# Twinklebear/tray_rust

Hardware: NVIDIA H100
Metric: Mrays/s (primary+secondary) (higher is better)
Workload: dtype f32

## Files before the change

include/trb.h:

```cpp
#ifndef TRB_H
#define TRB_H

#include <stdint.h>
#include <stddef.h>

#ifdef __cplusplus
extern "C" {
#endif

#define TRB_ABI_VERSION 4u

typedef enum trb_status {
    TRB_OK = 0,
    TRB_INVALID_ARG = 1,
    TRB_CUDA = 2,
    TRB_OOM = 3,
    TRB_UNSUPPORTED = 4,
    TRB_IO = 5,
    TRB_NO_DEVICE = 6,
    TRB_NCCL = 7
} trb_status;


typedef struct trb_keyframe {
// ... 590 lines not shown
                                     uint32_t* pixel_spp, trb_stats* stats);

trb_status trb_adaptive_schedule(const trb_adaptive* adaptive, uint32_t* min_spp, uint32_t* max_spp, uint32_t* step,
                                 uint32_t* max_per_pixel);

trb_status trb_host_adaptive_decide(const trb_adaptive* adaptive, const float* lum, size_t n, uint32_t* samples_taken,
                                    float* avg);


trb_status trb_block_list(const trb_scene* scene, uint32_t block_start, uint32_t block_count,
                          uint32_t* n_out, uint32_t* xy_pairs, uint32_t capacity);

trb_status trb_scene_get_bvh(const trb_scene* scene, int which, uint32_t* n_nodes, trb_bvh_node* nodes,
                             uint32_t* n_ordered, uint32_t* ordered);

trb_status trb_scene_get_transform(const trb_scene* scene, uint32_t inst, float* mat16, float* inv16);

trb_status trb_scene_get_filter_table(const trb_scene* scene, float* table256);


trb_status trb_host_build_bvh(const float* boxes6, uint32_t n, uint32_t max_geom, uint32_t* n_nodes,
                              trb_bvh_node* nodes, uint32_t* ordered);

trb_status trb_build_bvh(int device, const float* boxes6, uint32_t n, uint32_t max_geom, uint32_t* n_nodes,
                         trb_bvh_node* nodes, uint32_t* ordered);

trb_status trb_build_bvh_device(int device, const float* d_boxes6, uint32_t n, uint32_t max_geom, uint32_t* d_n_nodes,
                                trb_bvh_node* d_nodes, uint32_t* d_ordered, void* cuda_stream);

trb_status trb_host_keyframe_transform(const trb_keyframe* kf, float* mat16, float* inv16);
// ... 30 lines not shown
```

tray_rust_b200/_ffi.py:

```python
import ctypes as C
import os

_HERE = os.path.dirname(os.path.abspath(__file__))
REPO = os.path.dirname(_HERE)

TRB_ABI_VERSION = 4
TRB_OK, TRB_INVALID_ARG, TRB_CUDA, TRB_OOM, TRB_UNSUPPORTED, TRB_IO, TRB_NO_DEVICE, TRB_NCCL = range(8)
INST_RECEIVER, INST_EMITTER_AREA, INST_EMITTER_POINT = 0, 1, 2
SHAPE_NONE, SHAPE_SPHERE, SHAPE_DISK, SHAPE_RECT, SHAPE_MESH = 0, 1, 2, 3, 4
MAT_MATTE, MAT_PLASTIC, MAT_METAL, MAT_SPECULAR_METAL, MAT_GLASS, MAT_ROUGH_GLASS, MAT_MERL = range(7)
FILTER_MITCHELL_NETRAVALI, FILTER_GAUSSIAN = 0, 1
INTEGRATOR_PATH, INTEGRATOR_WHITTED, INTEGRATOR_NORMALS_DEBUG = 0, 1, 2
RENDER_STATS, RENDER_NO_UPDATE, RENDER_REFERENCE_SHADOW, RENDER_MEGAKERNEL, RENDER_TIME_TRACE = 1, 2, 4, 8, 16
QUERY_CLAMP = 32
BXDF_REFLECTION, BXDF_TRANSMISSION, BXDF_DIFFUSE, BXDF_GLOSSY, BXDF_SPECULAR = 1, 2, 4, 8, 16
BXDF_ALL = 31
MISS = 0xFFFFFFFF
BVH_LEAF = 0x80000000
MERL_TABLE_FLOATS = 90 * 90 * 180 * 3

u32, f32 = C.c_uint32, C.c_float


class Keyframe(C.Structure):
# ... 236 lines not shown
BSDF_SAMPLE_QUERY_DTYPE = np.dtype([("wo", "<f4", 3), ("bxdf", "<u4"), ("u", "<f4", 2), ("u_comp", "<f4"), ("pad", "<u4")])
BSDF_SAMPLE_DTYPE = np.dtype([("f", "<f4", 3), ("pdf", "<f4"), ("wi", "<f4", 3), ("sampled", "<u4")])
LIGHT_QUERY_DTYPE = np.dtype([("p", "<f4", 3), ("time", "<f4"), ("u", "<f4", 2), ("light", "<u4"), ("pad", "<u4")])
LIGHT_SAMPLE_DTYPE = np.dtype([("li", "<f4", 3), ("pdf", "<f4"), ("wi", "<f4", 3), ("delta", "<u4"), ("shadow", QUERY_RAY_DTYPE)])
LIGHT_PDF_QUERY_DTYPE = np.dtype([("p", "<f4", 3), ("time", "<f4"), ("wi", "<f4", 3), ("light", "<u4")])
EMIT_QUERY_DTYPE = np.dtype([("w", "<f4", 3), ("time", "<f4"), ("n", "<f4", 3), ("inst", "<u4")])
KEYFRAME_DTYPE = np.dtype([("translation", "<f4", 3), ("rotation", "<f4", 4), ("scaling", "<f4", 3)])
COLOR_KEY_DTYPE = np.dtype([("rgba", "<f4", 4), ("time", "<f4")])
AOV_SAMPLE_DTYPE = np.dtype([("albedo", "<f4", 3), ("depth", "<f4"), ("n", "<f4", 3), ("inst", "<u4")])
MATERIAL_DTYPE = np.dtype([("type", "<u4"), ("c0", "<f4", 3), ("c1", "<f4", 3), ("roughness", "<f4"), ("eta", "<f4"), ("merl", "<u4"),
                           ("tex", "<u4", 4)])

TRB_SYMBOLS = [
    "trb_scene_create", "trb_scene_load_json", "trb_scene_destroy", "trb_scene_info", "trb_scene_update_frame",
    "trb_render", "trb_render_device", "trb_intersect", "trb_intersect_device", "trb_camera_rays",
    "trb_render_samples", "trb_film_to_srgb8", "trb_block_list", "trb_scene_get_bvh", "trb_scene_get_transform",
    "trb_scene_get_filter_table", "trb_last_error", "trb_abi_version", "trb_desc_load_json", "trb_desc_free",
    "trb_host_build_bvh", "trb_host_keyframe_transform", "trb_host_animated_transform", "trb_host_animated_color", "trb_host_quad_check", "trb_selftest_box", "trb_launch_count", "trb_scene_trace_time", "trb_scene_check_error", "trb_scene_set_option", "trb_write_png",
    "trb_nccl_unique_id", "trb_comm_create", "trb_comm_destroy", "trb_comm_info", "trb_comm_reduce_film", "trb_render_sharded",
    "trb_group_create", "trb_group_load_json", "trb_group_render", "trb_group_scene", "trb_group_destroy",
    "trb_render_adaptive", "trb_render_samples_adaptive", "trb_adaptive_schedule", "trb_host_adaptive_decide",
    "trb_render_adaptive_device", "trb_render_sharded_adaptive", "trb_group_render_adaptive",
    "trb_intersect_records", "trb_intersect_records_device", "trb_occluded", "trb_occluded_device",
    "trb_illumination", "trb_illumination_device",
    "trb_bsdf_eval", "trb_bsdf_eval_device", "trb_bsdf_sample", "trb_bsdf_sample_device", "trb_light_sample", "trb_light_sample_device",
    "trb_light_pdf", "trb_light_pdf_device", "trb_emitted", "trb_emitted_device", "trb_scene_lights",
    "trb_film_write", "trb_film_write_device", "trb_camera_rays_device", "trb_host_film_to_srgb8",
    "trb_build_bvh", "trb_build_bvh_device",
    "trb_scene_update_mesh", "trb_scene_update_mesh_device", "trb_scene_refit_mesh", "trb_scene_refit_mesh_device",
    "trb_scene_update_keyframes", "trb_scene_update_keyframes_device", "trb_scene_update_color_keys", "trb_scene_update_materials",
    "trb_scene_replace_objects", "trb_scene_replace_meshes", "trb_scene_replace_meshes_device",
# ... 93 lines not shown
                                                 C.POINTER(DenoiseMomentsGradientOutput)]
    lib.trb_denoise_moments_gradient_device.argtypes = [vp, vp, C.POINTER(DenoiseFrame), C.POINTER(DenoiseGradientParams), u32,
                                                        C.POINTER(DenoiseMomentsGradientOutput), vp]
    lib.trb_render_adaptive.argtypes = [vp, C.POINTER(RenderCfg), C.POINTER(Adaptive), vp, vp, C.POINTER(Stats)]
    lib.trb_render_samples_adaptive.argtypes = [vp, C.POINTER(RenderCfg), C.POINTER(Adaptive), sz, vp, vp, C.POINTER(Stats)]
    lib.trb_render_adaptive_device.argtypes = [vp, C.POINTER(RenderCfg), C.POINTER(Adaptive), vp, vp, vp, vp]
    lib.trb_render_adaptive_aov.argtypes = [vp, C.POINTER(RenderCfg), C.POINTER(Adaptive), vp, C.POINTER(AovFilm), vp, C.POINTER(Stats)]
    lib.trb_render_adaptive_aov_device.argtypes = [vp, C.POINTER(RenderCfg), C.POINTER(Adaptive), vp, C.POINTER(AovFilm), vp, vp, vp]
    lib.trb_render_samples_adaptive_aov.argtypes = [vp, C.POINTER(RenderCfg), C.POINTER(Adaptive), sz, vp, vp, vp, C.POINTER(Stats)]
    lib.trb_adaptive_schedule.argtypes = [C.POINTER(Adaptive)] + [C.POINTER(u32)] * 4
    lib.trb_host_adaptive_decide.argtypes = [C.POINTER(Adaptive), vp, sz, C.POINTER(u32), C.POINTER(f32)]
    lib.trb_film_to_srgb8.argtypes = [vp, vp, vp]
    lib.trb_host_film_to_srgb8.argtypes = [u32, u32, vp, vp]
    lib.trb_block_list.argtypes = [vp, u32, u32, C.POINTER(u32), vp, u32]
    lib.trb_scene_get_bvh.argtypes = [vp, C.c_int, C.POINTER(u32), vp, C.POINTER(u32), vp]
    lib.trb_scene_get_transform.argtypes = [vp, u32, vp, vp]
    lib.trb_scene_get_filter_table.argtypes = [vp, vp]
    lib.trb_desc_load_json.argtypes = [C.c_char_p, u32, u32, u32, C.POINTER(C.POINTER(SceneDesc))]
    lib.trb_desc_free.argtypes = [C.POINTER(SceneDesc)]
    lib.trb_desc_free.restype = None
    lib.trb_host_build_bvh.argtypes = [vp, u32, u32, C.POINTER(u32), vp, vp]
    lib.trb_build_bvh.argtypes = [C.c_int, vp, u32, u32, C.POINTER(u32), vp, vp]
    lib.trb_build_bvh_device.argtypes = [C.c_int, vp, u32, u32, vp, vp, vp, vp]
    lib.trb_host_keyframe_transform.argtypes = [C.POINTER(Keyframe), vp, vp]
    lib.trb_host_animated_transform.argtypes = [C.POINTER(SceneDesc), u32, u32, f32, vp, vp]
    lib.trb_host_animated_color.argtypes = [C.POINTER(SceneDesc), u32, u32, f32, vp]
    lib.trb_host_quad_check.argtypes = [vp, u32, vp, u32, C.POINTER(u32), C.POINTER(C.c_uint64), C.POINTER(C.c_uint64)]
    lib.trb_selftest_box.argtypes = [u32, u32, C.POINTER(C.c_uint64)]
    lib.trb_launch_count.restype = C.c_uint64
    lib.trb_scene_trace_time.argtypes = [vp, C.POINTER(f32), C.POINTER(u32)]
# ... 26 lines not shown
```

tray_rust_b200/api.py:

```python
import ctypes as C

import numpy as np

from . import _ffi as F


class TrbError(RuntimeError):
    def __init__(self, status, msg):
        super().__init__("trb status %d: %s" % (status, msg))
        self.status = status


def _cfg(spp=0, sample_first=0, sample_count=0, block_start=0, block_count=0, current_frame=0, seed=1, flags=0,
         shard_index=0, shard_count=0, shard_chunk=0):
    return F.RenderCfg(spp, sample_first, sample_count, block_start, block_count, current_frame, seed, flags,
                       shard_index, shard_count, shard_chunk)


def adaptive_schedule(min_spp, max_spp):
    lib = F.load_trb()
    out = [F.u32() for _ in range(4)]
    rc = lib.trb_adaptive_schedule(C.byref(F.Adaptive(min_spp, max_spp)), *(C.byref(x) for x in out))
    if rc != F.TRB_OK:
        raise TrbError(rc, (lib.trb_last_error() or b"").decode())
# ... 537 lines not shown
            n = section.n_meshes
            meshes = (F.Mesh * max(1, n))()
            for i in range(n):
                k = section.keep[i]
                meshes[i] = section.meshes[i] if k == F.MESH_NEW else self._desc.meshes[k]
            desc.meshes, desc.n_meshes = meshes, n
        desc._keep = (self._desc, objects, section, meshes, materials)
        self._desc = desc
        w, hh, spp, nb, ni, nl = (F.u32() for _ in range(6))
        self._check(self._lib.trb_scene_info(self._h, *(C.byref(x) for x in (w, hh, spp, nb, ni, nl))))
        self.width, self.height, self.spp, self.total_blocks, self.n_instances, self.n_lights = (x.value for x in (w, hh, spp, nb, ni, nl))

    def set_option(self, name, value):
        self._check(self._lib.trb_scene_set_option(self._h, name.encode(), int(value)))

    def check_error(self):
        self._check(self._lib.trb_scene_check_error(self._h))

    def trace_time(self):
        ms, n = F.f32(), F.u32()
        self._check(self._lib.trb_scene_trace_time(self._h, C.byref(ms), C.byref(n)))
        return ms.value, n.value

    def render_samples(self, **kw):
        cfg = _cfg(**kw)
        n = self._n_samples(cfg)
        out = np.zeros(n, F.SAMPLE_DTYPE)
        st = F.Stats()
        self._check(self._lib.trb_render_samples(self._h, C.byref(cfg), n, F.ptr(out), C.byref(st)))
        return out, st
# ... 291 lines not shown
```

tray_rust_b200/csrc/trb_api.cu:

```cuda
#include <chrono>
#include <dlfcn.h>
#include <nccl.h>
#include <cstdio>
#include <cstdlib>
#include <memory>
#include <thread>
#include <tuple>
#include <cub/device/device_radix_sort.cuh>
#include "trb_host.h"
#include "trb_kernels.cuh"
#include "trb_bvh_build.cuh"
#include "trb_denoise.cuh"

using namespace trbh;

namespace {

thread_local std::string g_error;
unsigned long long g_launches = 0;
trb_status fail(trb_status s, const std::string& msg) { g_error = msg; return s; }

#define CU(call)                                                                                                   \
    do {                                                                                                           \
        cudaError_t e_ = (call);                                                                                   \
// ... 21 lines not shown
        if (e != cudaSuccess) return e;
        ptrs.push_back(d);
        *out = static_cast<T*>(d);
        return e;
    }
    void release(const void* p) {
        for (size_t i = 0; i < ptrs.size(); ++i)
            if (ptrs[i] == p) { cudaFree(ptrs[i]); ptrs[i] = ptrs.back(); ptrs.pop_back(); return; }
    }
};

struct HostMesh {
    std::vector<trb_bvh_node> nodes;
    std::vector<uint32_t> order;
    Box3 bounds;
    uint32_t n_verts = 0;
    bool narrow = true;
    size_t pair_cap = 0;
    bool stale = false;
    uint32_t* d_refit = nullptr;
};

uint32_t pow2_ceil(uint32_t v) { uint32_t p = 1; while (p < v) p <<= 1; return p; }

float bits_f(uint32_t u) { float f; std::memcpy(&f, &u, 4); return f; }
constexpr uint32_t QUAD_EMPTY_HOST = 0xffffffffu;
bool pack_pairs(const std::vector<trb_bvh_node>& in, std::vector<trb::DPair>& out, trb::DBvh& hdr, bool wide = false) {
    std::vector<uint32_t> rec_of(in.size(), 0);
    uint32_t n_rec = 0;
    for (size_t i = 0; i < in.size(); ++i) if (!(in[i].b & TRB_BVH_LEAF)) rec_of[i] = n_rec++;
    bool ok = n_rec < (1u << 30);
// ... 94 lines not shown
    int quads = 0;
    int exact_box = 0;
    int wide_leaf = 0;
    int pipe = 36;
    int film_v2 = 1;
    int sort = 0;
    int sort_bits = 5;
    int sort_min_round = 1;
    int shade_anim_occ = 4;
    int frame_device = 1;
    int anim_table = 2;
    int shade_split = -1;
    int shade_sort = 1;
    int shade_kind = 1;
    uint64_t pass_paths = 1ull << 24;
    int build_device = 1;
    long long tlas_min = -1;
    int frame_time = 0;
    int tlas_small = 8;
};
constexpr uint32_t kTlasLevelMin = 256;
int env_int(const char* name, int dflt) { const char* v = getenv(name); return v ? (int)strtol(v, nullptr, 0) : dflt; }
void tuning_from_env(Tuning& t) {
    t.refill = env_int("TRB_REFILL", t.refill); t.trace_grid = (unsigned)env_int("TRB_TRACE_GRID", (int)t.trace_grid);
    t.sched = (uint32_t)env_int("TRB_TRACE_SCHED", (int)t.sched); t.quads = env_int("TRB_TRACE_QUADS", t.quads); t.pipe = env_int("TRB_TRACE_PIPE", t.pipe);
    t.wide_leaf = env_int("TRB_TRACE_WIDE_LEAF", t.wide_leaf);
    t.film_v2 = env_int("TRB_FILM_V2", t.film_v2); t.sort = env_int("TRB_SORT", t.sort); t.sort_bits = env_int("TRB_SORT_BITS", t.sort_bits);
    t.sort_min_round = env_int("TRB_SORT_MIN_ROUND", t.sort_min_round); t.shade_split = env_int("TRB_SHADE_SPLIT", t.shade_split); t.anim_table = env_int("TRB_ANIM_TABLE", t.anim_table); t.frame_device = env_int("TRB_FRAME_DEVICE", t.frame_device);
    if (getenv("TRB_PASS_PATHS")) t.pass_paths = strtoull(getenv("TRB_PASS_PATHS"), nullptr, 0);
    t.build_device = env_int("TRB_BUILD_DEVICE", t.build_device);
    t.tlas_min = env_int("TRB_FRAME_TLAS_MIN", (int)t.tlas_min); t.frame_time = env_int("TRB_FRAME_TIME", t.frame_time);
    t.tlas_small = std::max(4, env_int("TRB_FRAME_TLAS_SMALL", t.tlas_small));
}

}

struct BlockList {
    uint32_t key[5];
    std::vector<uint32_t> host;
    uint2* dev = nullptr;
};

struct trb_scene {
    int device = 0;
    int sm_count = 0;
// ... 1152 lines not shown
        trb::DPair* out = nullptr;
        { const trb_status r = records(n_rec, &out); if (r != TRB_OK) return r; }
        trb::bvhb::k_pair_pack<<<grid(n), 256>>>(d_nodes, n, d_rec, wide, out, d_rec + n + 1);
        ++g_launches;
        CU(cudaGetLastError());
        uint32_t bad = 0;
        CU(cudaMemcpy(&bad, d_rec + n + 1, 4, cudaMemcpyDeviceToHost));
        *fits_narrow = bad == 0;
        return TRB_OK;
    };
    const trb_status r = run();
    cudaFree(d_rec); cudaFree(d_cub);
    return r;
}

trb_status setup_mesh(trb_scene* s, DeviceArena& arena, const trb_mesh& m, bool device, cudaStream_t st, HostMesh& hm, trb::DMesh& dm) {
    hm.n_verts = m.n_verts;
    float *dp, *dn, *dt; uint32_t* di; trb::DPair* dnodes; trb::DTri* dtris;
    const size_t nv = m.n_verts, ni = 3 * (size_t)m.n_tris;
    if (!device) {
        CU(arena.upload(m.positions, 3 * nv, &dp));
        CU(arena.upload(m.normals, 3 * nv, &dn));
        CU(arena.upload(m.texcoords, 2 * nv, &dt));
        CU(arena.upload(m.indices, ni, &di));
    } else {
        CU(arena.alloc(3 * nv, &dp)); CU(arena.alloc(3 * nv, &dn)); CU(arena.alloc(2 * nv, &dt)); CU(arena.alloc(ni, &di));
        uint32_t* d_bad = nullptr;
        CU(arena.alloc(1, &d_bad));
        CU(cudaMemcpyAsync(dp, m.positions, 3 * nv * sizeof(float), cudaMemcpyDeviceToDevice, st));
        CU(cudaMemcpyAsync(dn, m.normals, 3 * nv * sizeof(float), cudaMemcpyDeviceToDevice, st));
        CU(cudaMemcpyAsync(dt, m.texcoords, 2 * nv * sizeof(float), cudaMemcpyDeviceToDevice, st));
        CU(cudaMemcpyAsync(di, m.indices, ni * sizeof(uint32_t), cudaMemcpyDeviceToDevice, st));
// ... 18 lines not shown
    hdr.root_hi = make_float4(hm.bounds.hi[0], hm.bounds.hi[1], hm.bounds.hi[2], bits_f(QUAD_EMPTY_HOST));
    hm.narrow = leaves_fit_narrow(hm.nodes);
    if (hm.narrow) {
        std::vector<trb::DQuad> qn;
        uint32_t qroot = 0;
        if (!pack_quads(hm.nodes, qn, qroot)) return fail(TRB_UNSUPPORTED, "mesh too large for the leaf encoding (2^25 triangles)");
        hdr.root_hi.w = bits_f(qroot);
        trb::DQuad* dquads;
        CU(arena.upload(qn.data(), qn.size(), &dquads));
        hdr.quads = dquads;
    }
    CU(arena.alloc(n_rec, &dnodes));
    hm.pair_cap = n_rec;
    hdr.pairs = dnodes;
    dm.positions = dp; dm.normals = dn; dm.texcoords = dt; dm.indices = di; dm.tris = dtris;
    dm.n_nodes = (uint32_t)hm.nodes.size(); dm.n_tris = m.n_tris;
    return TRB_OK;
}

cudaError_t mesh_copy_in(const float* dst, const float* src, size_t n, bool device, cudaStream_t st) {
    if (!device) return cudaMemcpy(const_cast<float*>(dst), src, n * sizeof(float), cudaMemcpyHostToDevice);
    const cudaError_t e = cudaMemcpyAsync(const_cast<float*>(dst), src, n * sizeof(float), cudaMemcpyDeviceToDevice, st);
    return e != cudaSuccess ? e : cudaStreamSynchronize(st);
}
trb_status copy_mesh_attributes(trb_scene* s, uint32_t mi, const float* nrm, const float* uv, bool device, cudaStream_t st) {
    const trb::DMesh& dm = s->dmeshes[mi];
    const size_t nv = s->meshes[mi].n_verts;
    if (nrm) CU(mesh_copy_in(dm.normals, nrm, 3 * nv, device, st));
    if (uv) CU(mesh_copy_in(dm.texcoords, uv, 2 * nv, device, st));
    return TRB_OK;
}

// ... 19 lines not shown
        cudaEventSynchronize(ev.e[5]);
        static const char* const phase[5] = {"build", "read-back", "triangle records", "pack", "frame refresh"};
        for (int k = 0; k < 5; ++k) {
            float ms = 0.f;
            cudaEventElapsedTime(&ms, ev.e[k], ev.e[k + 1]);
            fprintf(stderr, "trb_scene_update_mesh %s %.3f ms\n", phase[k], ms);
        }
    };
    if (pos) {
        float* d_pos = nullptr;
        trb::DTri* d_tris = nullptr;
        trb_bvh_node* d_nodes = nullptr;
        HostMesh nm;
        auto build = [&]() -> trb_status {
            CU(s->arena.alloc(3 * nv, &d_pos));
            CU(s->arena.alloc(dm.n_tris, &d_tris));
            mark(0);
            CU(copy_in(d_pos, pos, 3 * nv));
            return build_mesh_bvh(s->tune.build_device != 0, d_pos, dm.indices, dm.n_tris, nm, d_tris, &d_nodes, ev.e[1], ev.e[2]);
        };
        { const trb_status r = build(); if (r != TRB_OK) { s->arena.release(d_pos); s->arena.release(d_tris); return r; } }
        mark(3);
        trb::DPair* pairs = const_cast<trb::DPair*>(dm.bvh.pairs);
        size_t cap = hm.pair_cap;
        auto records = [&](uint32_t n_rec, trb::DPair** out) -> trb_status {
            if (n_rec > cap) {
                trb::DPair* grown = nullptr;
                CU(s->arena.alloc(n_rec, &grown));
                pairs = grown; cap = n_rec;
            }
            *out = pairs;
            return TRB_OK;
        };
        bool narrow = true;
// ... 19 lines not shown
            return r;
        }
        mark(4);
        s->arena.release(dm.positions);
        s->arena.release(dm.tris);
        if (pairs != dm.bvh.pairs) s->arena.release(dm.bvh.pairs);
        if (dm.bvh.quads) s->arena.release(dm.bvh.quads);
        if (hm.d_refit) s->arena.release(hm.d_refit);
        hm.nodes = std::move(nm.nodes); hm.order = std::move(nm.order);
        hm.narrow = narrow; hm.pair_cap = cap; hm.stale = false; hm.d_refit = nullptr;
        for (int k = 0; k < 3; ++k) { hm.bounds.lo[k] = hm.nodes[0].bmin[k]; hm.bounds.hi[k] = hm.nodes[0].bmax[k]; }
        const trb_bvh_node& root = hm.nodes[0];
        uint32_t root_ref = trb::REF_INTERIOR;
        if (root.b & TRB_BVH_LEAF)
            root_ref = s->wide_leaf ? (trb::REF_LEAF | (root.a & ~trb::REF_TAG)) : (trb::REF_LEAF | ((root.b & ~TRB_BVH_LEAF) << 25) | root.a);
        dm.positions = d_pos; dm.tris = d_tris; dm.n_nodes = (uint32_t)hm.nodes.size();
        dm.bvh.pairs = pairs; dm.bvh.quads = nullptr;
        dm.bvh.root_lo = make_float4(hm.bounds.lo[0], hm.bounds.lo[1], hm.bounds.lo[2], bits_f(root_ref));
        dm.bvh.root_hi = make_float4(hm.bounds.hi[0], hm.bounds.hi[1], hm.bounds.hi[2], bits_f(QUAD_EMPTY_HOST));
        s->quads_dropped = true;
        s->needs_wide = false;
        for (const HostMesh& m : s->meshes) if (!m.narrow) s->needs_wide = true;
        const bool wide = s->needs_wide || s->tune.wide_leaf != 0;
        if (wide != s->wide_leaf) {
            const trb_status rw = upload_mesh_nodes(s, wide);
            if (rw != TRB_OK) return rw;
        } else CU(cudaMemcpy(s->d_meshes + mi, &dm, sizeof dm, cudaMemcpyHostToDevice));
    } else CU(cudaDeviceSynchronize());
    { const trb_status r = copy_mesh_attributes(s, mi, nrm, uv, device, st); if (r != TRB_OK) return r; }
    if (pos && s->frame_set) {
        const trb_status r = trb_scene_update_frame(s, s->last_frame, s->last_start, s->last_end);
        if (r != TRB_OK) return r;
    }
    report();
    return TRB_OK;
}

trb_status refit_mesh(trb_scene* s, uint32_t mi, const float* pos, const float* nrm, const float* uv, bool device, cudaStream_t st) {
    if (!pos) return update_mesh(s, mi, nullptr, nrm, uv, device, st);
    if (!s) return fail(TRB_INVALID_ARG, "null scene");
    if (mi >= s->meshes.size()) return fail(TRB_INVALID_ARG, "mesh index out of range");
    CU(cudaSetDevice(s->device));
    HostMesh& hm = s->meshes[mi];
    trb::DMesh& dm = s->dmeshes[mi];
// ... 2 lines not shown
    CU(cudaDeviceSynchronize());
    if (!hm.d_refit) {
        uint32_t* links = nullptr;
        CU(s->arena.alloc(2 * (size_t)n_rec, &links));
        hm.d_refit = links;
        trb::bvhb::k_refit_parents<<<grid(n_rec), 256, 0, st>>>(dm.bvh.pairs, n_rec, hm.d_refit);
        ++g_launches;
    }
    CU(mesh_copy_in(dm.positions, pos, 3 * (size_t)hm.n_verts, device, st));
    if (dm.bvh.quads) { s->arena.release(dm.bvh.quads); dm.bvh.quads = nullptr; }
    dm.bvh.root_hi.w = bits_f(QUAD_EMPTY_HOST);
    s->quads_dropped = true;
    trb::DMesh* d_dm = s->d_meshes + mi;
    CU(cudaMemcpyAsync(d_dm, &dm, sizeof dm, cudaMemcpyHostToDevice, st));
    if (n_rec) CU(cudaMemsetAsync(hm.d_refit + n_rec, 0, 4 * (size_t)n_rec, st));
    trb::bvhb::k_refit_tris<<<grid(dm.n_tris), 256, 0, st>>>(dm.positions, dm.indices, dm.n_tris, const_cast<trb::DTri*>(dm.tris));
    trb::bvhb::k_refit_nodes<<<grid(n_rec), 256, 0, st>>>(const_cast<trb::DPair*>(dm.bvh.pairs), n_rec, hm.d_refit, hm.d_refit + n_rec,
                                                          s->wide_leaf, dm.tris, dm.indices, dm.positions, &d_dm->bvh);
    g_launches += 2;
    CU(cudaGetLastError());
    trb::DBvh hdr{};
    CU(cudaMemcpyAsync(&hdr, &d_dm->bvh, sizeof hdr, cudaMemcpyDeviceToHost, st));
    CU(cudaStreamSynchronize(st));
    dm.bvh.root_lo = hdr.root_lo; dm.bvh.root_hi = hdr.root_hi;
    for (int k = 0; k < 3; ++k) { hm.bounds.lo[k] = (&hdr.root_lo.x)[k]; hm.bounds.hi[k] = (&hdr.root_hi.x)[k]; }
    hm.stale = true;
    { const trb_status r = copy_mesh_attributes(s, mi, nrm, uv, device, st); if (r != TRB_OK) return r; }
    if (s->frame_set) return trb_scene_update_frame(s, s->last_frame, s->last_start, s->last_end);
    return TRB_OK;
}

trb_status edit_check(const trb_scene* s, uint32_t first, uint32_t count, const void* a, size_t n, bool device, bool* done) {
    *done = false;
    if (!s) return fail(TRB_INVALID_ARG, "null scene");
    if (count == 0) { *done = true; return TRB_OK; }
    if (!a) return fail(TRB_INVALID_ARG, "null array");
    if ((uint64_t)first + count > n) return fail(TRB_INVALID_ARG, "edit range out of bounds");
    if (device && (reinterpret_cast<uintptr_t>(a) & 3u)) return fail(TRB_INVALID_ARG, "device array must be 4-byte aligned");
    return TRB_OK;
}

trb_status update_keyframes(trb_scene* s, uint32_t first, uint32_t count, const trb_keyframe* kf) {
// ... 210 lines not shown
    }
    const bool wide = needs_wide || s->tune.wide_leaf != 0, repack = wide != s->wide_leaf;
    if (!repack)
        for (uint32_t i = 0; i < n; ++i)
            if (sec.keep[i] == TRB_MESH_NEW) { const trb_status r = pack_mesh_nodes(built[i], dmeshes[i].bvh, wide); if (r != TRB_OK) return r; }
    trb::DMesh* d_meshes = nullptr;
    CU(fresh.upload(dmeshes.data(), dmeshes.size(), &d_meshes));
    StagedObjects g;
    if (o) { const trb_status r = stage_objects(s, *o, g); if (r != TRB_OK) return r; }

    CU(cudaDeviceSynchronize());
    for (uint32_t k = 0; k < n_old; ++k) {
        if (named[k]) continue;
        const trb::DMesh& dm = s->dmeshes[k];
        for (const void* p : {(const void*)dm.positions, (const void*)dm.normals, (const void*)dm.texcoords, (const void*)dm.indices,
                              (const void*)dm.tris, (const void*)dm.bvh.pairs, (const void*)dm.bvh.quads, (const void*)s->meshes[k].d_refit})
            if (p) s->arena.release(p);
    }
    s->arena.release(s->d_meshes);
    s->arena.ptrs.insert(s->arena.ptrs.end(), fresh.ptrs.begin(), fresh.ptrs.end());
    fresh.ptrs.clear();
    std::vector<HostMesh> meshes(n);
    for (uint32_t i = 0; i < n; ++i) meshes[i] = std::move(sec.keep[i] == TRB_MESH_NEW ? built[i] : s->meshes[sec.keep[i]]);
    s->meshes.swap(meshes); s->dmeshes.swap(dmeshes);
    s->d_meshes = d_meshes; s->ds.meshes = d_meshes;
    s->needs_wide = needs_wide;
    s->quads_dropped = false;
    for (uint32_t i = 0; i < n; ++i) if (s->meshes[i].narrow && !s->dmeshes[i].bvh.quads) s->quads_dropped = true;
    if (o) { commit_objects(s, g); objects_replaced(s); }
    else { s->instances_static_uploaded = false; s->frame_ready = false; }
    if (repack) { const trb_status r = upload_mesh_nodes(s, wide); if (r != TRB_OK) return r; }
// ... 258 lines not shown
    }
    else if (k == "trace.pipe") t.pipe = (int)value;
    else if (k == "trace.exact_box") t.exact_box = (int)value;
    else if (k == "trace.wide_leaf") {
        t.wide_leaf = (int)value;
        const bool wide = s->needs_wide || value != 0;
        if (wide != s->wide_leaf) { CU(cudaSetDevice(s->device)); return upload_mesh_nodes(s, wide); }
    }
    else if (k == "film.v2") t.film_v2 = (int)value;
    else if (k == "sort.mode") t.sort = (int)value;
    else if (k == "sort.bits") t.sort_bits = (int)std::min<long long>(6, std::max<long long>(1, value));
    else if (k == "sort.min_round") t.sort_min_round = (int)value;
    else if (k == "shade.split") t.shade_split = (int)value;
    else if (k == "shade.sort") t.shade_sort = (int)value;
    else if (k == "shade.kind") t.shade_kind = (int)value;
    else if (k == "anim.table") t.anim_table = (int)value;
    else if (k == "shade.anim_occupancy") t.shade_anim_occ = (int)value;
    else if (k == "pass.paths") { if (value < 64) return fail(TRB_INVALID_ARG, "pass.paths must be >= 64"); t.pass_paths = (uint64_t)value; }
    else return fail(TRB_INVALID_ARG, "unknown option: " + k);
    return TRB_OK;
}

trb_status trb_scene_check_error(trb_scene* s) {
    if (!s) return fail(TRB_INVALID_ARG, "null scene");
    CU(cudaSetDevice(s->device));
    CU(cudaDeviceSynchronize());
    return check_error_flag(s);
}

trb_status trb_scene_trace_time(trb_scene* s, float* total_ms, uint32_t* n_launches) {
// ... 1668 lines not shown
trb_status trb_host_film_to_srgb8(uint32_t width, uint32_t height, const float* film, uint8_t* rgb8) {
    const size_t npx = (size_t)width * height;
    if (npx && (!film || !rgb8)) return fail(TRB_INVALID_ARG, "null argument");
    for (size_t i = 0; i < npx; ++i) trb::srgb8_pixel(film[4 * i], film[4 * i + 1], film[4 * i + 2], film[4 * i + 3], rgb8 + 3 * i);
    return TRB_OK;
}

trb_status trb_block_list(const trb_scene* s, uint32_t start, uint32_t count, uint32_t* n_out, uint32_t* xy, uint32_t cap) {
    if (!s || !n_out) return fail(TRB_INVALID_ARG, "null argument");
    std::vector<uint32_t> b = morton_blocks(s->film.width, s->film.height, start, count);
    *n_out = (uint32_t)(b.size() / 2);
    if (xy) std::memcpy(xy, b.data(), sizeof(uint32_t) * std::min<size_t>(b.size(), 2 * (size_t)cap));
    return TRB_OK;
}

trb_status trb_scene_get_bvh(const trb_scene* s, int which, uint32_t* n_nodes, trb_bvh_node* nodes, uint32_t* n_ordered, uint32_t* ordered) {
    if (!s || !n_nodes || !n_ordered) return fail(TRB_INVALID_ARG, "null argument");
    const std::vector<trb_bvh_node>* nn; const std::vector<uint32_t>* oo;
    std::vector<trb_bvh_node> dev_nodes; std::vector<uint32_t> dev_order;
    if (which < 0) {
        if (!s->frame_ready) return fail(TRB_INVALID_ARG, "update_frame first");
        if (s->host_frame_stale) {
            CU(cudaSetDevice(s->device));
            dev_nodes.resize(s->tlas_n_nodes); dev_order.resize(s->instances.size());
            CU(cudaMemcpy(dev_nodes.data(), s->d_tlas_nodes, dev_nodes.size() * sizeof(trb_bvh_node), cudaMemcpyDeviceToHost));
            CU(cudaMemcpy(dev_order.data(), s->d_tlas_order, dev_order.size() * sizeof(uint32_t), cudaMemcpyDeviceToHost));
            nn = &dev_nodes; oo = &dev_order;
        } else { nn = &s->tlas_nodes; oo = &s->tlas_order; }
    }
    else {
// ... 549 lines not shown
```

tray_rust_b200/csrc/trb_bvh_build.cuh:

```cuda
#pragma once
#include <cub/device/device_scan.cuh>
#include "trb_device.h"
#include "trb_host.h"

namespace trb {
namespace bvhb {

constexpr uint32_t SMALL = 1024;
constexpr uint32_t NONE = 0xffffffffu;
enum : uint32_t { K_SAH = 0, K_LEAF = 1, K_KEEP = 2, K_PART = 3 };
enum : uint32_t { T_LEAF = 0, T_INTERIOR = 1, T_SMALL = 2 };

__device__ __forceinline__ float hmin(float a, float b) { if (isnan(a)) return b; if (isnan(b)) return a; return b < a ? b : a; }
__device__ __forceinline__ float hmax(float a, float b) { if (isnan(a)) return b; if (isnan(b)) return a; return b > a ? b : a; }
__device__ __forceinline__ void hgrow(trbh::Box3& b, const trbh::Box3& o) {
    for (int i = 0; i < 3; ++i) { b.lo[i] = hmin(b.lo[i], o.lo[i]); b.hi[i] = hmax(b.hi[i], o.hi[i]); }
}
__device__ __forceinline__ trbh::Box3 load_box(const float* boxes, uint32_t g) {
    trbh::Box3 b;
    for (int i = 0; i < 3; ++i) { b.lo[i] = boxes[6 * (size_t)g + i]; b.hi[i] = boxes[6 * (size_t)g + 3 + i]; }
    return b;
}
__device__ __forceinline__ uint32_t okey(float v) {
    const uint32_t u = __float_as_uint(v == 0.0f ? 0.0f : v);
// ... 374 lines not shown
__global__ void k_tri_pack(const float* __restrict__ pos, const uint32_t* __restrict__ tri, const uint32_t* __restrict__ order, uint32_t n_tris,
                           DTri* __restrict__ out) {
    const uint32_t slot = blockIdx.x * blockDim.x + threadIdx.x;
    if (slot >= n_tris) return;
    const uint32_t t = order[slot];
    const float* pa = pos + 3 * (size_t)tri[3 * (size_t)t];
    const float* pb = pos + 3 * (size_t)tri[3 * (size_t)t + 1];
    const float* pc = pos + 3 * (size_t)tri[3 * (size_t)t + 2];
    DTri r;
    r.v0 = make_float4(pa[0], pa[1], pa[2], __uint_as_float(t));
    r.e0 = make_float4(pb[0] - pa[0], pb[1] - pa[1], pb[2] - pa[2], 0.f);
    r.e1 = make_float4(pc[0] - pa[0], pc[1] - pa[1], pc[2] - pa[2], 0.f);
    r.pad = make_float4(0.f, 0.f, 0.f, 0.f);
    out[slot] = r;
}
__global__ void k_tri_leaf_marks(const trb_bvh_node* __restrict__ nodes, uint32_t n_nodes, DTri* tris) {
    const uint32_t i = blockIdx.x * blockDim.x + threadIdx.x;
    if (i >= n_nodes) return;
    const trb_bvh_node nd = nodes[i];
    const uint32_t cnt = nd.b & ~TRB_BVH_LEAF;
    if ((nd.b & TRB_BVH_LEAF) && cnt) tris[(size_t)nd.a + cnt - 1].e0.w = __uint_as_float(TRI_LEAF_END);
}
__global__ void k_mesh_index_check(const uint32_t* __restrict__ idx, size_t n, uint32_t n_verts, uint32_t* bad) {
    const size_t n4 = n / 4, stride = (size_t)gridDim.x * blockDim.x, t = blockIdx.x * (size_t)blockDim.x + threadIdx.x;
    const uint4* __restrict__ v = reinterpret_cast<const uint4*>(idx);
    bool out = false;
    for (size_t i = t; i < n4; i += stride) {
        const uint4 q = v[i];
        out |= (q.x >= n_verts) | (q.y >= n_verts) | (q.z >= n_verts) | (q.w >= n_verts);
    }
// ... 252 lines not shown
```

tray_rust_b200/csrc/trb_device.h:

```cpp
#pragma once
#include <cstdint>
#include <cuda_runtime.h>
#include "../../include/trb.h"
#include "trb_host.h"

namespace trb {

struct DNode { float4 lo, hi; };
constexpr uint32_t LEAF_BIT = 0x80000000u;

struct DPair {
    float4 l_lo;
    float4 l_hi;
    float4 r_lo;
    float4 r_hi;
};
constexpr uint32_t REF_TAG = 0xc0000000u, REF_INTERIOR = 0x00000000u, REF_LEAF = 0x40000000u;

struct DQuad { float4 q[8]; };
constexpr uint32_t QUAD_EMPTY = 0xffffffffu;

struct DBvh {
    const DPair* pairs;
    const DQuad* quads;
    float4 root_lo;
    float4 root_hi;
};
static_assert(sizeof(DBvh) == 48, "DBvh layout");

struct alignas(64) DTri { float4 v0, e0, e1, pad; };
static_assert(sizeof(DTri) == 64, "DTri layout");
constexpr uint32_t TRI_LEAF_END = 0xffffffffu;

struct DMesh {
    const float* positions;
    const float* normals;
    const float* texcoords;
    const uint32_t* indices;
    DBvh bvh;
    const DTri* tris;
    uint32_t n_nodes, n_tris;
};

struct alignas(16) DInstance {
    float inv[16];
    float mat[16];
    uint32_t kind, shape;
    float p0, p1;
    uint32_t mesh, material;
    float emission[3];
    uint32_t flags;
    uint32_t spline_first, n_splines;
    uint32_t emission_first, n_emission;
    uint32_t anim_slot;
    uint32_t pad;
    uint32_t xf_first, xf_count;
    uint32_t pad2[2];
// ... 89 lines not shown
```

tray_rust_b200/csrc/trb_kernels.cuh:

```cuda
#pragma once
#include "trb_device.h"
#include "trb_detmath.cuh"
#include "trb_anim.h"
#include "trb_adaptive.h"
#include "../../include/trb.h"

namespace trb {

struct f3 { float x, y, z; };
TRB_HD __forceinline__ f3 mk(float x, float y, float z) { f3 r; r.x = x; r.y = y; r.z = z; return r; }
__device__ __forceinline__ f3 splat(float v) { return mk(v, v, v); }
__device__ __forceinline__ f3 operator+(f3 a, f3 b) { return mk(a.x + b.x, a.y + b.y, a.z + b.z); }
__device__ __forceinline__ f3 operator-(f3 a, f3 b) { return mk(a.x - b.x, a.y - b.y, a.z - b.z); }
__device__ __forceinline__ f3 operator*(f3 a, f3 b) { return mk(a.x * b.x, a.y * b.y, a.z * b.z); }
__device__ __forceinline__ float ieee_div(float a, float b) { return a / b; }
__device__ __forceinline__ float ieee_sqrt(float a) { return sqrtf(a); }
__device__ __forceinline__ f3 operator/(f3 a, f3 b) { return mk(ieee_div(a.x, b.x), ieee_div(a.y, b.y), ieee_div(a.z, b.z)); }
__device__ __forceinline__ f3 operator*(f3 a, float s) { return mk(a.x * s, a.y * s, a.z * s); }
__device__ __forceinline__ f3 operator*(float s, f3 a) { return mk(s * a.x, s * a.y, s * a.z); }
__device__ __forceinline__ f3 operator/(f3 a, float s) { return mk(ieee_div(a.x, s), ieee_div(a.y, s), ieee_div(a.z, s)); }
__device__ __forceinline__ f3 operator-(f3 a) { return mk(-a.x, -a.y, -a.z); }
__device__ __forceinline__ float dot3(f3 a, f3 b) { return a.x * b.x + a.y * b.y + a.z * b.z; }
__device__ __forceinline__ f3 cross3(f3 a, f3 b) { return mk(a.y * b.z - a.z * b.y, a.z * b.x - a.x * b.z, a.x * b.y - a.y * b.x); }
__device__ __forceinline__ float len2(f3 a) { return a.x * a.x + a.y * a.y + a.z * a.z; }
// ... 589 lines not shown
    const LocalStack stack{stack_mem};
    trace_init(sc, t, ray, any_hit, time);
    while (t.cur != ST_DONE) trace_step<STATS, ANIM, WIDE>(sc, t, stack, cnt, err);
    ray.tmax = t.tmax;
    hit.t = t.tmax; hit.inst = t.h_inst; hit.prim = t.h_prim; hit.b1 = t.h_b1; hit.b2 = t.h_b2;
    return t.found;
}

struct Surf { f3 p, n, ng, dp_du; float u, v; };

template <bool ANIM, bool RECORD = false>
__device__ __forceinline__ void surface_at(const DScene& sc, const Ray& ray, const HitRec& hit, Surf& s, float time, const float* xf_row = nullptr,
                                           f3* dp_dv_world = nullptr) {
    const DInstance& in = sc.instances[hit.inst];
    float m[16], w[16];
    instance_inv_mat<ANIM>(sc, in, time, m, w, xf_row);
    const f3 o = xf_point(m, ray.o), d = xf_vector(m, ray.d);
    const f3 p = o + d * hit.t;
    const uint32_t shape = __ldg(&in.shape);
    f3 n, ng, dp_du;
    f3 dp_dv_rec;
    if (shape == TRB_SHAPE_MESH) {
        const DMesh& me = sc.meshes[__ldg(&in.mesh)];
        const uint32_t ia = __ldg(&me.indices[3 * hit.prim]), ib = __ldg(&me.indices[3 * hit.prim + 1]), ic = __ldg(&me.indices[3 * hit.prim + 2]);
        const float* P = me.positions; const float* N = me.normals; const float* T = me.texcoords;
        const f3 pa = mk(__ldg(P + 3 * ia), __ldg(P + 3 * ia + 1), __ldg(P + 3 * ia + 2));
        const f3 pb = mk(__ldg(P + 3 * ib), __ldg(P + 3 * ib + 1), __ldg(P + 3 * ib + 2));
        const f3 pc = mk(__ldg(P + 3 * ic), __ldg(P + 3 * ic + 1), __ldg(P + 3 * ic + 2));
        const f3 na = mk(__ldg(N + 3 * ia), __ldg(N + 3 * ia + 1), __ldg(N + 3 * ia + 2));
        const f3 nb = mk(__ldg(N + 3 * ib), __ldg(N + 3 * ib + 1), __ldg(N + 3 * ib + 2));
        const f3 nc = mk(__ldg(N + 3 * ic), __ldg(N + 3 * ic + 1), __ldg(N + 3 * ic + 2));
        const float b1 = hit.b1, b2 = hit.b2;
        const float b0 = 1.0f - b1 - b2;
        n = unit(unit(b0 * na + b1 * nb + b2 * nc));
        ng = n;
        const float tax = __ldg(T + 2 * ia), tay = __ldg(T + 2 * ia + 1), tbx = __ldg(T + 2 * ib), tby = __ldg(T + 2 * ib + 1);
        const float tcx = __ldg(T + 2 * ic), tcy = __ldg(T + 2 * ic + 1);
        s.u = b0 * tax + b1 * tbx + b2 * tcx; s.v = b0 * tay + b1 * tby + b2 * tcy;
        const float du0 = tax - tcx, du1 = tbx - tcx, dv0 = tay - tcy, dv1 = tby - tcy;
        const float det = du0 * dv1 - dv0 * du1;
        if (det == 0.0f) {
            f3 dp_dv;
            coord_system(unit(cross3(pc - pa, pb - pa)), dp_du, dp_dv);
            if (RECORD) dp_dv_rec = dp_dv;
        } else {
            const float idet = 1.0f / det;
            const f3 dp0 = pa - pc, dp1 = pb - pc;
            dp_du = (dv1 * dp0 - dv0 * dp1) * idet;
            if (RECORD) dp_dv_rec = (-du1 * dp0 + du0 * dp1) * idet;
        }
    } else if (shape == TRB_SHAPE_SPHERE) {
        n = unit(p); ng = n;
// ... 19 lines not shown
        if (RECORD) dp_dv_rec = dp_dv;
        if (RECORD || sc.n_textures) {
            float phi = datan2(p.y, p.x);
            if (phi < 0.0f) phi += TRB_PI * 2.0f;
            s.u = phi / (2.0f * TRB_PI); s.v = 1.0f - (hr - inner) / (radius - inner);
        }
    } else {
        const float hw = __ldg(&in.p0) / 2.0f, hh = __ldg(&in.p1) / 2.0f;
        dp_du = mk(hw * 2.0f, 0.0f, 0.0f);
        const f3 dp_dv = mk(0.0f, hh * 2.0f, 0.0f);
        n = unit(cross3(dp_du, dp_dv));
        ng = unit(mk(0.0f, 0.0f, 1.0f));
        if (RECORD) dp_dv_rec = dp_dv;
        s.u = (p.x + hw) / (2.0f * hw); s.v = (p.y + hh) / (2.0f * hh);
    }
    s.p = xf_point(w, p);
    s.n = xf_normal_t(m, n);
    s.ng = xf_normal_t(m, ng);
    s.dp_du = xf_vector(w, dp_du);
    if (RECORD) *dp_dv_world = xf_vector(w, dp_dv_rec);
}

__device__ __forceinline__ void concentric_disk(float u0, float u1, float& ox, float& oy) {
    float s0 = 2.0f * u0 - 1.0f, s1 = 2.0f * u1 - 1.0f;
    if (s0 == 0.0f && s1 == 0.0f) { ox = s0; oy = s1; return; }
    float radius, theta;
    if (s0 >= -s1) {
        if (s0 > s1) { radius = s0; theta = s1 > 0.0f ? ieee_div(s1, s0) : 8.0f + ieee_div(s1, s0); }
        else { radius = s1; theta = 2.0f - ieee_div(s0, s1); }
    } else if (s0 <= s1) { radius = -s0; theta = 4.0f + ieee_div(s1, s0); }
// ... 2413 lines not shown
```

Before: 780.3.

## Precompute per-triangle shading records and skip animated transform for static instances

Adds a per-mesh array of 96-byte triangle records (positions, normals, UVs packed into six float4s), filled by a new kernel at mesh setup, update and refit. The hit-shading path then reads six vectorized loads instead of index lookups followed by scattered scalar vertex loads. Shading also now skips the animated-transform evaluation when an instance has no animated transform flag. The cost is extra device memory per triangle, with a guard against low free memory, and an extra fill pass whenever meshes change. The DMesh header drops n_nodes/n_tris to stay 96 bytes.

```diff
diff --git a/include/trb.h b/include/trb.h
--- a/include/trb.h
+++ b/include/trb.h
@@ -628,6 +628,8 @@
 trb_status trb_scene_get_bvh(const trb_scene* scene, int which, uint32_t* n_nodes, trb_bvh_node* nodes,
                              uint32_t* n_ordered, uint32_t* ordered);
 
+trb_status trb_scene_get_shade_records(const trb_scene* scene, uint32_t mesh, uint32_t* n_records, float* records);
+
 trb_status trb_scene_get_transform(const trb_scene* scene, uint32_t inst, float* mat16, float* inv16);
 
 trb_status trb_scene_get_filter_table(const trb_scene* scene, float* table256);
diff --git a/tray_rust_b200/_ffi.py b/tray_rust_b200/_ffi.py
--- a/tray_rust_b200/_ffi.py
+++ b/tray_rust_b200/_ffi.py
@@ -274,7 +274,7 @@
 TRB_SYMBOLS = [
     "trb_scene_create", "trb_scene_load_json", "trb_scene_destroy", "trb_scene_info", "trb_scene_update_frame",
     "trb_render", "trb_render_device", "trb_intersect", "trb_intersect_device", "trb_camera_rays",
-    "trb_render_samples", "trb_film_to_srgb8", "trb_block_list", "trb_scene_get_bvh", "trb_scene_get_transform",
+    "trb_render_samples", "trb_film_to_srgb8", "trb_block_list", "trb_scene_get_bvh", "trb_scene_get_shade_records", "trb_scene_get_transform",
     "trb_scene_get_filter_table", "trb_last_error", "trb_abi_version", "trb_desc_load_json", "trb_desc_free",
     "trb_host_build_bvh", "trb_host_keyframe_transform", "trb_host_animated_transform", "trb_host_animated_color", "trb_host_quad_check", "trb_selftest_box", "trb_launch_count", "trb_scene_trace_time", "trb_scene_check_error", "trb_scene_set_option", "trb_write_png",
     "trb_nccl_unique_id", "trb_comm_create", "trb_comm_destroy", "trb_comm_info", "trb_comm_reduce_film", "trb_render_sharded",
@@ -398,6 +398,7 @@
     lib.trb_host_film_to_srgb8.argtypes = [u32, u32, vp, vp]
     lib.trb_block_list.argtypes = [vp, u32, u32, C.POINTER(u32), vp, u32]
     lib.trb_scene_get_bvh.argtypes = [vp, C.c_int, C.POINTER(u32), vp, C.POINTER(u32), vp]
+    lib.trb_scene_get_shade_records.argtypes = [vp, u32, C.POINTER(u32), vp]
     lib.trb_scene_get_transform.argtypes = [vp, u32, vp, vp]
     lib.trb_scene_get_filter_table.argtypes = [vp, vp]
     lib.trb_desc_load_json.argtypes = [C.c_char_p, u32, u32, u32, C.POINTER(C.POINTER(SceneDesc))]
diff --git a/tray_rust_b200/api.py b/tray_rust_b200/api.py
--- a/tray_rust_b200/api.py
+++ b/tray_rust_b200/api.py
@@ -575,6 +575,16 @@
     def set_option(self, name, value):
         self._check(self._lib.trb_scene_set_option(self._h, name.encode(), int(value)))
 
+    def shade_records(self, mesh):
+        n = F.u32()
+        f = self._lib.trb_scene_get_shade_records
+        self._check(f(self._h, mesh, C.byref(n), None))
+        if n.value == 0:
+            return None
+        out = np.zeros((n.value, 24), np.float32)
+        self._check(f(self._h, mesh, C.byref(n), F.ptr(out)))
+        return out
+
     def check_error(self):
         self._check(self._lib.trb_scene_check_error(self._h))
 
diff --git a/tray_rust_b200/csrc/trb_api.cu b/tray_rust_b200/csrc/trb_api.cu
--- a/tray_rust_b200/csrc/trb_api.cu
+++ b/tray_rust_b200/csrc/trb_api.cu
@@ -59,7 +59,7 @@
     std::vector<trb_bvh_node> nodes;
     std::vector<uint32_t> order;
     Box3 bounds;
-    uint32_t n_verts = 0;
+    uint32_t n_verts = 0, n_tris = 0;
     bool narrow = true;
     size_t pair_cap = 0;
     bool stale = false;
@@ -184,6 +184,7 @@
     int shade_sort = 1;
     int shade_kind = 1;
     uint64_t pass_paths = 1ull << 24;
+    int shade_records = 1;
     int build_device = 1;
     long long tlas_min = -1;
     int frame_time = 0;
@@ -199,6 +200,7 @@
     t.sort_min_round = env_int("TRB_SORT_MIN_ROUND", t.sort_min_round); t.shade_split = env_int("TRB_SHADE_SPLIT", t.shade_split); t.anim_table = env_int("TRB_ANIM_TABLE", t.anim_table); t.frame_device = env_int("TRB_FRAME_DEVICE", t.frame_device);
     if (getenv("TRB_PASS_PATHS")) t.pass_paths = strtoull(getenv("TRB_PASS_PATHS"), nullptr, 0);
     t.build_device = env_int("TRB_BUILD_DEVICE", t.build_device);
+    t.shade_records = env_int("TRB_SHADE_RECORDS", t.shade_records);
     t.tlas_min = env_int("TRB_FRAME_TLAS_MIN", (int)t.tlas_min); t.frame_time = env_int("TRB_FRAME_TIME", t.frame_time);
     t.tlas_small = std::max(4, env_int("TRB_FRAME_TLAS_SMALL", t.tlas_small));
 }
@@ -1381,8 +1383,38 @@
     return r;
 }
 
+trb_status shade_records_fill(const trb::DMesh& dm, uint32_t n_tris) {
+    if (!dm.shade) return TRB_OK;
+    trb::bvhb::k_shade_tris<<<(unsigned)(((size_t)n_tris + 255) / 256), 256>>>(dm.positions, dm.normals, dm.texcoords, dm.indices, n_tris,
+                                                                                const_cast<trb::DShadeTri*>(dm.shade));
+    ++g_launches;
+    CU(cudaGetLastError());
+    CU(cudaDeviceSynchronize());
+    return TRB_OK;
+}
+trb_status shade_records_setup(trb_scene* s, DeviceArena& arena, trb::DMesh& dm, uint32_t n_tris) {
+    if (!s->tune.shade_records || dm.shade) return shade_records_fill(dm, n_tris);
+    size_t free_b = 0, total_b = 0;
+    CU(cudaMemGetInfo(&free_b, &total_b));
+    if ((size_t)n_tris * sizeof(trb::DShadeTri) + total_b / 4 > free_b) return TRB_OK;
+    trb::DShadeTri* rec = nullptr;
+    CU(arena.alloc(n_tris, &rec));
+    dm.shade = rec;
+    return shade_records_fill(dm, n_tris);
+}
+trb_status set_shade_records(trb_scene* s) {
+    CU(cudaDeviceSynchronize());
+    for (size_t mi = 0; mi < s->dmeshes.size(); ++mi) {
+        trb::DMesh& dm = s->dmeshes[mi];
+        if (!s->tune.shade_records) { if (dm.shade) s->arena.release(dm.shade); dm.shade = nullptr; }
+        else { const trb_status r = shade_records_setup(s, s->arena, dm, s->meshes[mi].n_tris); if (r != TRB_OK) return r; }
+    }
+    if (!s->dmeshes.empty()) CU(cudaMemcpy(s->d_meshes, s->dmeshes.data(), s->dmeshes.size() * sizeof(trb::DMesh), cudaMemcpyHostToDevice));
+    return TRB_OK;
+}
+
 trb_status setup_mesh(trb_scene* s, DeviceArena& arena, const trb_mesh& m, bool device, cudaStream_t st, HostMesh& hm, trb::DMesh& dm) {
-    hm.n_verts = m.n_verts;
+    hm.n_verts = m.n_verts; hm.n_tris = m.n_tris;
     float *dp, *dn, *dt; uint32_t* di; trb::DPair* dnodes; trb::DTri* dtris;
     const size_t nv = m.n_verts, ni = 3 * (size_t)m.n_tris;
     if (!device) {
@@ -1431,8 +1463,8 @@
     hm.pair_cap = n_rec;
     hdr.pairs = dnodes;
     dm.positions = dp; dm.normals = dn; dm.texcoords = dt; dm.indices = di; dm.tris = dtris;
-    dm.n_nodes = (uint32_t)hm.nodes.size(); dm.n_tris = m.n_tris;
-    return TRB_OK;
+    dm.shade = nullptr;
+    return shade_records_setup(s, arena, dm, m.n_tris);
 }
 
 cudaError_t mesh_copy_in(const float* dst, const float* src, size_t n, bool device, cudaStream_t st) {
@@ -1482,10 +1514,10 @@
         HostMesh nm;
         auto build = [&]() -> trb_status {
             CU(s->arena.alloc(3 * nv, &d_pos));
-            CU(s->arena.alloc(dm.n_tris, &d_tris));
+            CU(s->arena.alloc(hm.n_tris, &d_tris));
             mark(0);
             CU(copy_in(d_pos, pos, 3 * nv));
-            return build_mesh_bvh(s->tune.build_device != 0, d_pos, dm.indices, dm.n_tris, nm, d_tris, &d_nodes, ev.e[1], ev.e[2]);
+            return build_mesh_bvh(s->tune.build_device != 0, d_pos, dm.indices, hm.n_tris, nm, d_tris, &d_nodes, ev.e[1], ev.e[2]);
         };
         { const trb_status r = build(); if (r != TRB_OK) { s->arena.release(d_pos); s->arena.release(d_tris); return r; } }
         mark(3);
@@ -1535,7 +1567,7 @@
         uint32_t root_ref = trb::REF_INTERIOR;
         if (root.b & TRB_BVH_LEAF)
             root_ref = s->wide_leaf ? (trb::REF_LEAF | (root.a & ~trb::REF_TAG)) : (trb::REF_LEAF | ((root.b & ~TRB_BVH_LEAF) << 25) | root.a);
-        dm.positions = d_pos; dm.tris = d_tris; dm.n_nodes = (uint32_t)hm.nodes.size();
+        dm.positions = d_pos; dm.tris = d_tris;
         dm.bvh.pairs = pairs; dm.bvh.quads = nullptr;
         dm.bvh.root_lo = make_float4(hm.bounds.lo[0], hm.bounds.lo[1], hm.bounds.lo[2], bits_f(root_ref));
         dm.bvh.root_hi = make_float4(hm.bounds.hi[0], hm.bounds.hi[1], hm.bounds.hi[2], bits_f(QUAD_EMPTY_HOST));
@@ -1549,6 +1581,7 @@
         } else CU(cudaMemcpy(s->d_meshes + mi, &dm, sizeof dm, cudaMemcpyHostToDevice));
     } else CU(cudaDeviceSynchronize());
     { const trb_status r = copy_mesh_attributes(s, mi, nrm, uv, device, st); if (r != TRB_OK) return r; }
+    { const trb_status r = shade_records_fill(dm, hm.n_tris); if (r != TRB_OK) return r; }
     if (pos && s->frame_set) {
         const trb_status r = trb_scene_update_frame(s, s->last_frame, s->last_start, s->last_end);
         if (r != TRB_OK) return r;
@@ -1581,7 +1614,7 @@
     trb::DMesh* d_dm = s->d_meshes + mi;
     CU(cudaMemcpyAsync(d_dm, &dm, sizeof dm, cudaMemcpyHostToDevice, st));
     if (n_rec) CU(cudaMemsetAsync(hm.d_refit + n_rec, 0, 4 * (size_t)n_rec, st));
-    trb::bvhb::k_refit_tris<<<grid(dm.n_tris), 256, 0, st>>>(dm.positions, dm.indices, dm.n_tris, const_cast<trb::DTri*>(dm.tris));
+    trb::bvhb::k_refit_tris<<<grid(hm.n_tris), 256, 0, st>>>(dm.positions, dm.indices, hm.n_tris, const_cast<trb::DTri*>(dm.tris));
     trb::bvhb::k_refit_nodes<<<grid(n_rec), 256, 0, st>>>(const_cast<trb::DPair*>(dm.bvh.pairs), n_rec, hm.d_refit, hm.d_refit + n_rec,
                                                           s->wide_leaf, dm.tris, dm.indices, dm.positions, &d_dm->bvh);
     g_launches += 2;
@@ -1593,6 +1626,7 @@
     for (int k = 0; k < 3; ++k) { hm.bounds.lo[k] = (&hdr.root_lo.x)[k]; hm.bounds.hi[k] = (&hdr.root_hi.x)[k]; }
     hm.stale = true;
     { const trb_status r = copy_mesh_attributes(s, mi, nrm, uv, device, st); if (r != TRB_OK) return r; }
+    { const trb_status r = shade_records_fill(dm, hm.n_tris); if (r != TRB_OK) return r; }
     if (s->frame_set) return trb_scene_update_frame(s, s->last_frame, s->last_start, s->last_end);
     return TRB_OK;
 }
@@ -1833,7 +1867,8 @@
         if (named[k]) continue;
         const trb::DMesh& dm = s->dmeshes[k];
         for (const void* p : {(const void*)dm.positions, (const void*)dm.normals, (const void*)dm.texcoords, (const void*)dm.indices,
-                              (const void*)dm.tris, (const void*)dm.bvh.pairs, (const void*)dm.bvh.quads, (const void*)s->meshes[k].d_refit})
+                              (const void*)dm.tris, (const void*)dm.bvh.pairs, (const void*)dm.bvh.quads, (const void*)s->meshes[k].d_refit,
+                              (const void*)dm.shade})
             if (p) s->arena.release(p);
     }
     s->arena.release(s->d_meshes);
@@ -2122,6 +2157,11 @@
     else if (k == "shade.split") t.shade_split = (int)value;
     else if (k == "shade.sort") t.shade_sort = (int)value;
     else if (k == "shade.kind") t.shade_kind = (int)value;
+    else if (k == "shade.records") {
+        const bool changed = (t.shade_records != 0) != (value != 0);
+        t.shade_records = (int)value;
+        if (changed) { CU(cudaSetDevice(s->device)); return set_shade_records(s); }
+    }
     else if (k == "anim.table") t.anim_table = (int)value;
     else if (k == "shade.anim_occupancy") t.shade_anim_occ = (int)value;
     else if (k == "pass.paths") { if (value < 64) return fail(TRB_INVALID_ARG, "pass.paths must be >= 64"); t.pass_paths = (uint64_t)value; }
@@ -3820,6 +3860,19 @@
     return TRB_OK;
 }
 
+trb_status trb_scene_get_shade_records(const trb_scene* s, uint32_t mesh, uint32_t* n_records, float* records) {
+    if (!s || !n_records) return fail(TRB_INVALID_ARG, "null argument");
+    if (mesh >= s->dmeshes.size()) return fail(TRB_INVALID_ARG, "mesh index out of range");
+    const trb::DMesh& dm = s->dmeshes[mesh];
+    const uint32_t n_tris = s->meshes[mesh].n_tris;
+    *n_records = dm.shade ? n_tris : 0u;
+    if (records && dm.shade) {
+        CU(cudaSetDevice(s->device));
+        CU(cudaMemcpy(records, dm.shade, (size_t)n_tris * sizeof(trb::DShadeTri), cudaMemcpyDeviceToHost));
+    }
+    return TRB_OK;
+}
+
 trb_status trb_scene_get_bvh(const trb_scene* s, int which, uint32_t* n_nodes, trb_bvh_node* nodes, uint32_t* n_ordered, uint32_t* ordered) {
     if (!s || !n_nodes || !n_ordered) return fail(TRB_INVALID_ARG, "null argument");
     const std::vector<trb_bvh_node>* nn; const std::vector<uint32_t>* oo;
diff --git a/tray_rust_b200/csrc/trb_bvh_build.cuh b/tray_rust_b200/csrc/trb_bvh_build.cuh
--- a/tray_rust_b200/csrc/trb_bvh_build.cuh
+++ b/tray_rust_b200/csrc/trb_bvh_build.cuh
@@ -412,6 +412,22 @@
     r.pad = make_float4(0.f, 0.f, 0.f, 0.f);
     out[slot] = r;
 }
+__global__ void k_shade_tris(const float* __restrict__ pos, const float* __restrict__ nrm, const float* __restrict__ uv,
+                             const uint32_t* __restrict__ tri, uint32_t n_tris, DShadeTri* __restrict__ out) {
+    const uint32_t t = blockIdx.x * blockDim.x + threadIdx.x;
+    if (t >= n_tris) return;
+    const size_t ia = tri[3 * (size_t)t], ib = tri[3 * (size_t)t + 1], ic = tri[3 * (size_t)t + 2];
+    const float *pa = pos + 3 * ia, *pb = pos + 3 * ib, *pc = pos + 3 * ic, *na = nrm + 3 * ia, *nb = nrm + 3 * ib, *nc = nrm + 3 * ic;
+    const float *ta = uv + 2 * ia, *tb = uv + 2 * ib, *tc = uv + 2 * ic;
+    DShadeTri r;
+    r.q[0] = make_float4(pa[0], pa[1], pa[2], pb[0]);
+    r.q[1] = make_float4(pb[1], pb[2], pc[0], pc[1]);
+    r.q[2] = make_float4(pc[2], na[0], na[1], na[2]);
+    r.q[3] = make_float4(nb[0], nb[1], nb[2], nc[0]);
+    r.q[4] = make_float4(nc[1], nc[2], ta[0], ta[1]);
+    r.q[5] = make_float4(tb[0], tb[1], tc[0], tc[1]);
+    out[t] = r;
+}
 __global__ void k_tri_leaf_marks(const trb_bvh_node* __restrict__ nodes, uint32_t n_nodes, DTri* tris) {
     const uint32_t i = blockIdx.x * blockDim.x + threadIdx.x;
     if (i >= n_nodes) return;
diff --git a/tray_rust_b200/csrc/trb_device.h b/tray_rust_b200/csrc/trb_device.h
--- a/tray_rust_b200/csrc/trb_device.h
+++ b/tray_rust_b200/csrc/trb_device.h
@@ -32,6 +32,9 @@
 static_assert(sizeof(DTri) == 64, "DTri layout");
 constexpr uint32_t TRI_LEAF_END = 0xffffffffu;
 
+struct DShadeTri { float4 q[6]; };
+static_assert(sizeof(DShadeTri) == 96, "DShadeTri layout");
+
 struct DMesh {
     const float* positions;
     const float* normals;
@@ -39,8 +42,9 @@
     const uint32_t* indices;
     DBvh bvh;
     const DTri* tris;
-    uint32_t n_nodes, n_tris;
+    const DShadeTri* shade;
 };
+static_assert(sizeof(DMesh) == 96, "DMesh layout: the trace kernels index the header array");
 
 struct alignas(16) DInstance {
     float inv[16];
diff --git a/tray_rust_b200/csrc/trb_kernels.cuh b/tray_rust_b200/csrc/trb_kernels.cuh
--- a/tray_rust_b200/csrc/trb_kernels.cuh
+++ b/tray_rust_b200/csrc/trb_kernels.cuh
@@ -627,7 +627,9 @@
                                            f3* dp_dv_world = nullptr) {
     const DInstance& in = sc.instances[hit.inst];
     float m[16], w[16];
-    instance_inv_mat<ANIM>(sc, in, time, m, w, xf_row);
+    const bool xf_anim = ANIM && (__ldg(&in.flags) & DI_ANIM_XF);
+    if (xf_anim) instance_inv_mat<ANIM>(sc, in, time, m, w, xf_row);
+    else load_xf(in.inv, m);
     const f3 o = xf_point(m, ray.o), d = xf_vector(m, ray.d);
     const f3 p = o + d * hit.t;
     const uint32_t shape = __ldg(&in.shape);
@@ -635,20 +637,31 @@
     f3 dp_dv_rec;
     if (shape == TRB_SHAPE_MESH) {
         const DMesh& me = sc.meshes[__ldg(&in.mesh)];
-        const uint32_t ia = __ldg(&me.indices[3 * hit.prim]), ib = __ldg(&me.indices[3 * hit.prim + 1]), ic = __ldg(&me.indices[3 * hit.prim + 2]);
-        const float* P = me.positions; const float* N = me.normals; const float* T = me.texcoords;
-        const f3 pa = mk(__ldg(P + 3 * ia), __ldg(P + 3 * ia + 1), __ldg(P + 3 * ia + 2));
-        const f3 pb = mk(__ldg(P + 3 * ib), __ldg(P + 3 * ib + 1), __ldg(P + 3 * ib + 2));
-        const f3 pc = mk(__ldg(P + 3 * ic), __ldg(P + 3 * ic + 1), __ldg(P + 3 * ic + 2));
-        const f3 na = mk(__ldg(N + 3 * ia), __ldg(N + 3 * ia + 1), __ldg(N + 3 * ia + 2));
-        const f3 nb = mk(__ldg(N + 3 * ib), __ldg(N + 3 * ib + 1), __ldg(N + 3 * ib + 2));
-        const f3 nc = mk(__ldg(N + 3 * ic), __ldg(N + 3 * ic + 1), __ldg(N + 3 * ic + 2));
+        const DShadeTri* R = me.shade;
+        f3 pa, pb, pc, na, nb, nc;
+        float tax, tay, tbx, tby, tcx, tcy;
+        if (R) {
+            const float4* q = R[hit.prim].q;
+            const float4 q0 = __ldg(q), q1 = __ldg(q + 1), q2 = __ldg(q + 2), q3 = __ldg(q + 3), q4 = __ldg(q + 4), q5 = __ldg(q + 5);
+            pa = mk(q0.x, q0.y, q0.z); pb = mk(q0.w, q1.x, q1.y); pc = mk(q1.z, q1.w, q2.x);
+            na = mk(q2.y, q2.z, q2.w); nb = mk(q3.x, q3.y, q3.z); nc = mk(q3.w, q4.x, q4.y);
+            tax = q4.z; tay = q4.w; tbx = q5.x; tby = q5.y; tcx = q5.z; tcy = q5.w;
+        } else {
+            const uint32_t ia = __ldg(&me.indices[3 * hit.prim]), ib = __ldg(&me.indices[3 * hit.prim + 1]), ic = __ldg(&me.indices[3 * hit.prim + 2]);
+            const float* P = me.positions; const float* N = me.normals; const float* T = me.texcoords;
+            pa = mk(__ldg(P + 3 * ia), __ldg(P + 3 * ia + 1), __ldg(P + 3 * ia + 2));
+            pb = mk(__ldg(P + 3 * ib), __ldg(P + 3 * ib + 1), __ldg(P + 3 * ib + 2));
+            pc = mk(__ldg(P + 3 * ic), __ldg(P + 3 * ic + 1), __ldg(P + 3 * ic + 2));
+            na = mk(__ldg(N + 3 * ia), __ldg(N + 3 * ia + 1), __ldg(N + 3 * ia + 2));
+            nb = mk(__ldg(N + 3 * ib), __ldg(N + 3 * ib + 1), __ldg(N + 3 * ib + 2));
+            nc = mk(__ldg(N + 3 * ic), __ldg(N + 3 * ic + 1), __ldg(N + 3 * ic + 2));
+            tax = __ldg(T + 2 * ia); tay = __ldg(T + 2 * ia + 1); tbx = __ldg(T + 2 * ib); tby = __ldg(T + 2 * ib + 1);
+            tcx = __ldg(T + 2 * ic); tcy = __ldg(T + 2 * ic + 1);
+        }
         const float b1 = hit.b1, b2 = hit.b2;
         const float b0 = 1.0f - b1 - b2;
         n = unit(unit(b0 * na + b1 * nb + b2 * nc));
         ng = n;
-        const float tax = __ldg(T + 2 * ia), tay = __ldg(T + 2 * ia + 1), tbx = __ldg(T + 2 * ib), tby = __ldg(T + 2 * ib + 1);
-        const float tcx = __ldg(T + 2 * ic), tcy = __ldg(T + 2 * ic + 1);
         s.u = b0 * tax + b1 * tbx + b2 * tcx; s.v = b0 * tay + b1 * tby + b2 * tcy;
         const float du0 = tax - tcx, du1 = tbx - tcx, dv0 = tay - tcy, dv1 = tby - tcy;
         const float det = du0 * dv1 - dv0 * du1;
@@ -698,6 +711,7 @@
         if (RECORD) dp_dv_rec = dp_dv;
         s.u = (p.x + hw) / (2.0f * hw); s.v = (p.y + hh) / (2.0f * hh);
     }
+    if (!xf_anim) load_xf(in.mat, w);
     s.p = xf_point(w, p);
     s.n = xf_normal_t(m, n);
     s.ng = xf_normal_t(m, ng);
```

Result: faster. 788.6, median of 6 (+1.1%).
